# genomicepidemiology/ccphylo

Measured on AMD Instinct MI355X. Metric: taxa-pairs/sec (dist) + NJ iterations/sec at N taxa, 1/2/4/8 MI355X, higher is better.
Workload: dtype u2 packed codes -> MX-fp4 MFMA (exact integer counts), f64 LT and tree

## Files before the change

ccphylo_amd/csrc/ccg_dnj_search.h:

```cpp
#pragma once
#include <stdlib.h>
#include "ccg_tree_common.h"

struct DenseRows {
	__host__ __device__ __forceinline__ bool owns(long long) const { return true; }
	__host__ __device__ __forceinline__ long long row(long long r) const { return tri(r); }
};

#define DNJ_B 128
#define DNJ_BANDS 64
#define DNJ_BANDS_MAX 128
#define SEG 2048
#define SEG_S 1024
#define SEL_RPL 8
#define SEL_STEPS 8
#define TBF 1024
#define FIND_RPT 16
#define FIND_CHUNKS 2048
#define REPLAY_CAP 2048
#define JOIN_UPRE 2048
#define FOLD_BLOCKS 256
#define PLAN_MAXB 256
#define SRDY_REP 64
#define UHIST 64
// ... 116 lines not shown
			const bool take = c < c1 && 0 <= d && qarg_better(x, c, q, idx);
			q = take ? x : q;
			idx = take ? c : idx;
		}
		if(more) {
#pragma unroll
			for(int m = 0; m < UNR; ++m) {
				v[m] = vn[m];
				nk[m] = nkn[m];
				sk[m] = skn[m];
			}
		}
	}
}

__device__ __forceinline__ void fold_units(const double *__restrict__ uq, const int *__restrict__ uj, int ua, int ub,
                                           double &q, int &idx) {
	for(int u = ua; u < ub; u += 4) {
		double oq[4];
		int oi[4];
#pragma unroll
		for(int m = 0; m < 4; ++m) {
			const int v = u + m < ub ? u + m : ub - 1;
			oq[m] = uq[v];
			oi[m] = uj[v];
		}
#pragma unroll
		for(int m = 0; m < 4; ++m) {
			if(u + m < ub && qarg_better(oq[m], oi[m], q, idx)) {
				q = oq[m];
				idx = oi[m];
			}
		}
	}
}

__device__ __forceinline__ void qarg_block_reduce1(double &q, int &idx, double *sq, int *si) {
	qarg_wave_reduce(q, idx);
	const int lane = threadIdx.x & 63, wid = threadIdx.x >> 6, nw = blockDim.x >> 6;
	if(lane == 0) {
		sq[wid] = q;
		si[wid] = idx;
	}
	__syncthreads();
	if(threadIdx.x == 0) {
		for(int w = 1; w < nw; ++w) {
			if(qarg_better(sq[w], si[w], q, idx)) {
				q = sq[w];
				idx = si[w];
			}
		}
	}
}

template <int ET, class Rows>
__global__ void k_init_hnj(Rows rows, const typename Elem<ET>::T *__restrict__ D, int n, double bs,
                           const double *__restrict__ sD, const int *__restrict__ N,
                           double *__restrict__ Q, int *__restrict__ P) {
	int i = blockIdx.x * (blockDim.x >> 6) + (threadIdx.x >> 6);
	int lane = threadIdx.x & 63;
	if(i >= n || !rows.owns(i)) return;
	double bq = DBL_MAX, bd = DBL_MAX;
	int bj = 0;
	const typename Elem<ET>::T *row = D + rows.row(i);
	int Ni = N[i];
	double sDi = sD[i];
	for(int j = lane; j < i; j += 64) {
		double d = Elem<ET>::get(row[j], bs);
		const double q = qcrit(Ni, N[j], d, sDi, sD[j]);
		const bool take = (0 <= d) & ((q < bq) | ((q == bq) & ((d < bd) | ((d == bd) & (j > bj)))));
		bq = take ? q : bq;
		bd = take ? d : bd;
		bj = take ? j : bj;
	}
#pragma unroll
	for(int off = 32; off > 0; off >>= 1) {
		const double oq = __shfl_xor(bq, off, 64), od = __shfl_xor(bd, off, 64);
		const int oj = __shfl_xor(bj, off, 64);
		const bool take = (oq < bq) | ((oq == bq) & ((od < bd) | ((od == bd) & (oj > bj))));
		bq = take ? oq : bq;
		bd = take ? od : bd;
		bj = take ? oj : bj;
	}
	if(lane == 0) {
		Q[i] = bq;
		P[i] = bj;
	}
}

template <int UNUSED = 0>
__global__ __launch_bounds__(TB) void k_dnj_prep(TreeBufs b, int n) {
	__shared__ double sq[TB / 64];
	__shared__ int si[TB / 64];
	double q = DBL_MAX;
	int idx = 0;
	for(int i = 1 + threadIdx.x; i < n; i += blockDim.x) {
		if(qarg_better(b.Q[i], i, q, idx)) {
			q = b.Q[i];
			idx = i;
		}
	}
	qarg_block_reduce(q, idx, sq, si);
	if(threadIdx.x == 0) {
		b.ctl->cand = idx;
		b.ctl->cand_q = b.Q[idx];
		b.ctl->cand_p = b.P[idx];
	}
}

__device__ __forceinline__ void s_table_h(const TreeBufs &b, int n, int nS, double m0) {
	const int lane = threadIdx.x & 63;
	double v[2];
#pragma unroll
	for(int h = 0; h < 2; ++h) {
		const int t = lane + 64 * h;
		v[h] = DBL_MAX;
		if(t < nS) {
			const double f = __hip_atomic_load(b.sfq + t, __ATOMIC_RELAXED, __HIP_MEMORY_SCOPE_AGENT);
			const double qt = __hip_atomic_load(b.pS_q + t, __ATOMIC_RELAXED, __HIP_MEMORY_SCOPE_AGENT);
			v[h] = f > qt ? f : qt;
		}
	}
	double x0 = wave_incl_min(v[0]);
	x0 = x0 < m0 ? x0 : m0;
	const double c = readlane_d(x0, 63);
	double x1 = wave_incl_min(v[1]);
	x1 = x1 < c ? x1 : c;
	if(lane < nS) __hip_atomic_store(b.pS_bnd + lane, x0, __ATOMIC_RELAXED, __HIP_MEMORY_SCOPE_AGENT);
	if(lane + 64 < nS) __hip_atomic_store(b.pS_bnd + lane + 64, x1, __ATOMIC_RELAXED, __HIP_MEMORY_SCOPE_AGENT);
	if(b.ctl->vtag == n) {
		const int G = (int) cdiv(n + 1, TB);
		double carry = DBL_MAX;
		for(int g1 = ((G - 1) / 64) * 64; g1 >= 0; g1 -= 64) {
			const int g = g1 + 63 - lane;
			double x = g < G ? b.bmv[g] : DBL_MAX;
			x = wave_incl_min(x);
			x = x < carry ? x : carry;
			if(g < G) __hip_atomic_store(b.vsuf + g, x, __ATOMIC_RELAXED, __HIP_MEMORY_SCOPE_AGENT);
			carry = readlane_d(x, 63);
		}
		if(lane == 0) __hip_atomic_store(b.vsuf + G, DBL_MAX, __ATOMIC_RELAXED, __HIP_MEMORY_SCOPE_AGENT);
	}
	asm volatile("s_waitcnt vmcnt(0)" ::: "memory");
	if(lane < SRDY_REP)
		__hip_atomic_store(b.srdy + 32 * lane, (unsigned) n, __ATOMIC_RELAXED, __HIP_MEMORY_SCOPE_AGENT);
}

#ifndef LB_BB_D
#define LB_BB_D 8
#endif
#ifndef LB_BB_N
#define LB_BB_N 8
#endif
template <int ET>
__device__ __forceinline__ int lb_unit(const typename Elem<ET>::T *__restrict__ row, double bs, const TreeBufs &b, int n,
                                       int r, int c0, int c1, double sDr, double &q, int &idx, int isub = -1,
                                       double sDm = 0.0, bool ubinf = false);

template <int ET>
__device__ __forceinline__ void plan_s_helper(const typename Elem<ET>::T *__restrict__ D, double bs,
                                                        TreeBufs b, int n, int hb, int nh, bool tshort) {
	typedef typename Elem<ET>::T T;
	constexpr int UC = 8;
	__shared__ int h_ok, h_nS, h_isub, h_jsub;
	__shared__ double h_m0, h_sDm;
	__shared__ int h_uo[DNJ_B + 1], h_row[DNJ_B];
	const int tid = threadIdx.x, lane = tid & 63, wid = tid >> 6;
	if(b.ctl->done) return;
	if(tid == 0) {
		bool ok = false;
		for(int spin = 0; spin < (tshort ? 1 << 10 : 1 << 18); ++spin) {
			if(__hip_atomic_load(b.shdr + 3, __ATOMIC_RELAXED, __HIP_MEMORY_SCOPE_AGENT) == (unsigned long long) n) {
				ok = true;
				break;
			}
			__builtin_amdgcn_s_sleep(4);
		}
		h_ok = ok;
		if(!ok) {
			b.ctl->final_n = -1;
			b.ctl->done = 1;
		}
		if(ok) {
			h_m0 = __longlong_as_double(
			    (long long) __hip_atomic_load(b.shdr + 0, __ATOMIC_RELAXED, __HIP_MEMORY_SCOPE_AGENT));
			h_sDm = __longlong_as_double(
			    (long long) __hip_atomic_load(b.shdr + 1, __ATOMIC_RELAXED, __HIP_MEMORY_SCOPE_AGENT));
			const unsigned long long w = __hip_atomic_load(b.shdr + 2, __ATOMIC_RELAXED, __HIP_MEMORY_SCOPE_AGENT);
			h_nS = (int) (unsigned) (w & 0xffffffffu);
			h_isub = (int) (unsigned) (w >> 32);
			h_jsub = (int) (unsigned) __hip_atomic_load(b.shdr + 4, __ATOMIC_RELAXED, __HIP_MEMORY_SCOPE_AGENT);
		}
	}
	__syncthreads();
	if(!h_ok || h_nS <= 0) return;
	const int nS = h_nS, isub = h_isub, jsub = h_jsub;
	const double sDm = h_sDm;
	for(int t = tid; t <= nS; t += blockDim.x) {
		h_uo[t] = __hip_atomic_load(b.pS_uo + t, __ATOMIC_RELAXED, __HIP_MEMORY_SCOPE_AGENT);
		if(t < nS) h_row[t] = __hip_atomic_load(b.pS_row + t, __ATOMIC_RELAXED, __HIP_MEMORY_SCOPE_AGENT);
	}
	__syncthreads();
	const int su = h_uo[nS];
	const int nwv = blockDim.x >> 6;
	for(int v = hb * nwv + wid; v < su; v += nh * nwv) {
		int lo = 0, hi = nS;
		while(hi - lo > 1) {
			const int mid = (lo + hi) >> 1;
			if(h_uo[mid] <= v) lo = mid; else hi = mid;
		}
		const int r = h_row[lo], c0 = (v - h_uo[lo]) * SEG_S;
		const int c1 = c0 + SEG_S < r ? c0 + SEG_S : r;
		const double sDr = r == isub ? sDm : b.sD[r];
		const T *row = D + tri(r);
		double q = DBL_MAX;
		int idx = 0;
		if(b.lbm) {
			const long long sk = lb_unit<ET>(row, bs, b, n, r, c0, c1, sDr, q, idx, isub, sDm, r == isub || r == jsub);
			if(lane == 0 && sk) {
				long long *slot = b.lbskip + (long long) (LB_SCAN + (hb * nwv + wid) % LB_HELP) * LB_SLOT;
				atomicAdd((unsigned long long *) slot, (unsigned long long) sk);
				atomicAdd((unsigned long long *) (slot + 1), (unsigned long long) sk);
			}
		} else {
			for(int base = c0; base < c1; base += 64 * UC) {
				double sk[UC];
				T vv[UC];
#pragma unroll
				for(int m = 0; m < UC; ++m) {
					const int c = base + 64 * m + lane;
					const int cc = c < c1 ? c : c1 - 1;
					sk[m] = b.sD[cc];
					vv[m] = row[cc];
				}
#pragma unroll
				for(int m = 0; m < UC; ++m) {
					const int c = base + 64 * m + lane;
					const double d = Elem<ET>::get(vv[m], bs);
					const double x = qcrit(n, n, d, sDr, c == isub ? sDm : sk[m]);
					const bool take = c < c1 && 0 <= d && qarg_better(x, c, q, idx);
					q = take ? x : q;
					idx = take ? c : idx;
				}
			}
		}
		qarg_wave_reduce(q, idx);
		int s_done = 0;
		const int ua = h_uo[lo], ub = h_uo[lo + 1];
		int last = 1;
		if(ub - ua > 1) {
			if(lane == 0) {
				__hip_atomic_store(b.uq + v, q, __ATOMIC_RELAXED, __HIP_MEMORY_SCOPE_AGENT);
				__hip_atomic_store(b.uj + v, idx, __ATOMIC_RELAXED, __HIP_MEMORY_SCOPE_AGENT);
				asm volatile("s_waitcnt vmcnt(0)" ::: "memory");
				const unsigned seen = __hip_atomic_fetch_add(b.ecS + lo, 1u, __ATOMIC_RELAXED, __HIP_MEMORY_SCOPE_AGENT);
				last = (int) seen == ub - ua - 1;
				if(last) __hip_atomic_store(b.ecS + lo, 0u, __ATOMIC_RELAXED, __HIP_MEMORY_SCOPE_AGENT);
			}
			last = __shfl(last, 0);
			if(last) {
				for(int x = ua + lane; x < ub; x += 64) {
					const double oq = __hip_atomic_load(b.uq + x, __ATOMIC_RELAXED, __HIP_MEMORY_SCOPE_AGENT);
					const int oi = __hip_atomic_load(b.uj + x, __ATOMIC_RELAXED, __HIP_MEMORY_SCOPE_AGENT);
					if(qarg_better(oq, oi, q, idx)) {
						q = oq;
						idx = oi;
					}
				}
				qarg_wave_reduce(q, idx);
			}
		}
		if(lane == 0) {
			if(last) {
				__hip_atomic_store(b.sfq + lo, q, __ATOMIC_RELAXED, __HIP_MEMORY_SCOPE_AGENT);
				__hip_atomic_store(b.sfj + lo, idx, __ATOMIC_RELAXED, __HIP_MEMORY_SCOPE_AGENT);
				asm volatile("s_waitcnt vmcnt(0)" ::: "memory");
				const unsigned sseen = __hip_atomic_fetch_add(&b.ctl->scnt, 1u, __ATOMIC_RELAXED, __HIP_MEMORY_SCOPE_AGENT);
				s_done = (int) sseen == nS - 1;
				if(s_done) __hip_atomic_store(&b.ctl->scnt, 0u, __ATOMIC_RELAXED, __HIP_MEMORY_SCOPE_AGENT);
			}
		}
		if(__shfl(s_done, 0)) s_table_h(b, n, nS, h_m0);
	}
}

template <int ET, bool GEN, class Rows, bool BANDS>
__global__ __launch_bounds__(TBF) void k_dnj_plan(const typename Elem<ET>::T *__restrict__ D, double bs, TreeBufs b,
                                                  int n, int first, Rows rows, int seg, int ktop, int kbands,
                                                  int qdelay) {
	constexpr int NW = TBF / 64, FR = FIND_RPT, NSP = TBF - 64, LT = TBF - 64, LW = NW - 1;
	__shared__ int sS[DNJ_B];
	__shared__ double sQS[DNJ_B], sQP[DNJ_B];
	__shared__ double spq[NSP];
	__shared__ double spm[DNJ_B + 2];
	__shared__ int s_mw[FR * LW], s_cnt;
	__shared__ double s_sb[LW * FR];
	__shared__ __attribute__((aligned(16))) unsigned char s_sf[LW * FR];
	__shared__ int sch[FIND_CHUNKS];
	__shared__ int s_done, s_isub, s_jsub, s_nS, s_ntop, s_smin, s_Nm;
	__shared__ double s_m0, s_Qj, s_Qi, s_sDm;
	TreeCtl *ctl = b.ctl;
	const int tid = threadIdx.x, lane = tid & 63, wid = tid >> 6;
	const int top = n - 1;
	const int fr = ((qdelay >> 17) & 15) + 1;
	const int nhelp = (qdelay >> 22) & 511;
	if((int) blockIdx.x >= (int) gridDim.x - nhelp) {
// ... 1934 lines not shown
```

ccphylo_amd/csrc/snp.hip:

```cpp
#include <cstring>
#include <vector>
#include <type_traits>
#include "ccg_internal.h"
#include "ccg_shard_layout.h"

#define TILE 128
#define KC 16
#define KCP 8
#define RS 130
#define RSP 130

__device__ __forceinline__ uint32_t xor_or(uint32_t a, uint32_t b, uint32_t c) {
	return __builtin_amdgcn_bitop3_b32(a, b, c, 0xBE);
}

__device__ __forceinline__ uint32_t compress_even(uint64_t x) {
	x &= 0x5555555555555555ull;
	x = (x | (x >> 1)) & 0x3333333333333333ull;
	x = (x | (x >> 2)) & 0x0F0F0F0F0F0F0F0Full;
	x = (x | (x >> 4)) & 0x00FF00FF00FF00FFull;
	x = (x | (x >> 8)) & 0x0000FFFF0000FFFFull;
	x = (x | (x >> 16)) & 0x00000000FFFFFFFFull;
	return (uint32_t) x;
}
// ... 470 lines not shown
				g0[x] = fp4_spread(b[x].x);
			}
#pragma unroll
			for(int ta = 0; ta < 4; ++ta)
#pragma unroll
				for(int tb = 0; tb < 4; ++tb)
					acc[ta][tb] = __builtin_amdgcn_mfma_scale_f32_32x32x64_f8f6f4(
					    f0[ta], g0[tb], acc[ta][tb], MFMA_FP4, MFMA_FP4, 0, MFMA_SCALE1, 0, MFMA_SCALE1);
#pragma unroll
			for(int x = 0; x < 4; ++x) {
				f1[x] = fp4_spread(a[x].y);
				g1[x] = fp4_spread(b[x].y);
			}
#pragma unroll
			for(int ta = 0; ta < 4; ++ta)
#pragma unroll
				for(int tb = 0; tb < 4; ++tb)
					acc[ta][tb] = __builtin_amdgcn_mfma_scale_f32_32x32x64_f8f6f4(
					    f1[ta], g1[tb], acc[ta][tb], MFMA_FP4, MFMA_FP4, 0, MFMA_SCALE1, 0, MFMA_SCALE1);
#pragma unroll
			for(int x = 0; x < 4; ++x) {
				f0[x] = fp4_xor_spread(f0[x], f1[x]);
				g0[x] = fp4_xor_spread(g0[x], g1[x]);
			}
#pragma unroll
			for(int ta = 0; ta < 4; ++ta)
#pragma unroll
				for(int tb = 0; tb < 4; ++tb)
					acc[ta][tb] = __builtin_amdgcn_mfma_scale_f32_32x32x64_f8f6f4(
					    f0[ta], g0[tb], acc[ta][tb], MFMA_FP4, MFMA_FP4, 0, MFMA_SCALE1, 0, MFMA_SCALE1);
		}
		if(more) {
			uint2 *An = As[buf ^ 1], *Bn = Bs[buf ^ 1];
#pragma unroll
			for(int q = 0; q < QS2; ++q) {
				const int e = q * 256 + threadIdx.x, row = e / WPR, wp = e % WPR;
				An[(2 * wp) * RS2 + row] = make_uint2(va[q].x, va[q].y);
				An[(2 * wp + 1) * RS2 + row] = make_uint2(va[q].z, va[q].w);
				Bn[(2 * wp) * RS2 + row] = make_uint2(vb[q].x, vb[q].y);
				Bn[(2 * wp + 1) * RS2 + row] = make_uint2(vb[q].z, vb[q].w);
			}
		}
		__syncthreads();
	}
	const int L3 = 3 * 32 * Wl;
#pragma unroll
	for(int ta = 0; ta < 4; ++ta) {
#pragma unroll
		for(int r = 0; r < 16; ++r) {
			const int l = 128 * wr + 32 * ta + (r & 3) + 8 * (r >> 2) + 4 * h;
			const long long L = (long long) I * TILE2 + l;
			long long i = L;
			if(BAND) {
				const long long lb = L / SB;
				i = (lb * world + rank) * SB + (L - lb * SB);
			}
			if(i >= n || (!BAND && (i < rowBegin || i >= rowEnd))) continue;
			const long long base = BAND ? sh.off(i) : tri(i);
#pragma unroll
			for(int tb = 0; tb < 4; ++tb) {
				const long long j = (long long) J * TILE2 + 128 * wc + 32 * tb + l32;
				if(j < i) {
					const unsigned d = (unsigned) ((L3 - (int) acc[ta][tb][r]) >> 2);
					if(SPLIT) {
						atomicAdd(&cnt[base + j - cbase], d);
					} else {
						const double v = nFactor * (double) d;
						D[base + j] = Elem<ET>::put(v, 0.5, bs);
					}
				}
			}
		}
	}
}

#define NST3 4
#define KC3 8
#ifdef CCG_DIST_STAMPS
#define ST3_SLOTS 8
__device__ unsigned long long *ccg_dist_stamp_buf;
__device__ long long ccg_dist_stamp_item0;
#define ST3(K)                                                                              \
	do {                                                                                    \
		unsigned long long tn_;                                                             \
		__builtin_amdgcn_sched_barrier(0);                                                  \
		asm volatile("s_memtime %0\n\ts_waitcnt lgkmcnt(0)" : "=s"(tn_)::"memory");         \
		__builtin_amdgcn_sched_barrier(0);                                                  \
		if((K) >= 0) stamp_sum[(K) < 0 ? 0 : (K)] += tn_ - stamp_prev;                      \
		stamp_prev = tn_;                                                                   \
	} while(0)
#else
#define ST3(K)
#endif
template <int ET, bool SPLIT, bool BAND>
__global__ __launch_bounds__(256, 1) void k_snp_mfma3(const uint2 *__restrict__ P, int Wp, int n, long long t0,
                                                      long long items, int S, int Wk, double nFactor, double bs,
                                                      typename Elem<ET>::T *__restrict__ D, long long rowBegin,
                                                      long long rowEnd, unsigned *__restrict__ cnt, long long cbase,
                                                      const long long *__restrict__ pfx, int npanels, int rank,
                                                      int world, int sorder) {
	constexpr int NSL = KC3 / 2;
	static_assert(NSL == 4, "one slice per wave");
	__shared__ __attribute__((aligned(16))) uint4 L[NST3 * 2 * NSL * TILE2];
	const long long item = t0 + xcd_tile(blockIdx.x, items), t = SPLIT ? item / S : item;
	int I, J;
	if(BAND) {
		int lo = 0, hi = npanels - 1;
		while(lo < hi) {
			const int mid = (lo + hi + 1) >> 1;
			if(pfx[mid] <= t) lo = mid; else hi = mid - 1;
		}
		I = lo;
		J = (int) (t - pfx[lo]);
	} else if(sorder) {
		tile_ij_super(t, (rowEnd - 1) / TILE2, I, J);
	} else {
		tile_ij(t, I, J);
	}
	const int wb = SPLIT ? (int) (item % S) * Wk : 0;
	const int Wl = SPLIT ? (wb + Wk < Wp ? Wk : Wp - wb) : Wp;
	const Shard sh{rank, world};
	const int lane = threadIdx.x & 63, wid = threadIdx.x >> 6;
	const uint2 *srcA[4], *srcB[4];
#pragma unroll
	for(int q = 0; q < 4; ++q) {
		const long long Lr = (long long) I * TILE2 + q * 64 + lane;
		long long r = Lr;
		if(BAND) {
			const long long lb = Lr / SB;
			r = (lb * world + rank) * SB + (Lr - lb * SB);
			r = r < n ? r : 0;
		}
		srcA[q] = P + (size_t) r * Wp + wb + 2 * wid;
		srcB[q] = P + ((size_t) J * TILE2 + q * 64 + lane) * Wp + wb + 2 * wid;
	}
	const int nch = Wl / KC3;
	const unsigned lbase = (unsigned) (uintptr_t) (__attribute__((address_space(3))) uint4 *) L;
	auto glds = [&](const uint2 *src, unsigned lds) {
		unsigned keep;
		asm volatile("s_mov_b32 %0, m0\n\ts_mov_b32 m0, %2\n\ts_nop 0\n\tglobal_load_lds_dwordx4 %1, off\n\ts_mov_b32 m0, %0"
		             : "=&s"(keep)
		             : "v"(src), "s"(lds)
		             : "memory");
	};
	const unsigned lwave = (unsigned) __builtin_amdgcn_readfirstlane((int) (lbase + (unsigned) (wid * TILE2 * 16)));
	auto issue1 = [&](int c, int i) {
		const int st = c % NST3, w0 = c * KC3, q = i >> 1, p = i & 1;
		glds((p ? srcB[q] : srcA[q]) + w0, lwave + (unsigned) ((((st * 2 + p) * NSL) * TILE2 + q * 64) * 16));
	};
	auto issue = [&](int c) {
#pragma unroll
		for(int i = 0; i < 8; ++i) issue1(c, i);
	};
	const int wr = wid >> 1, wc = wid & 1;
	const int h = lane >> 5, l32 = lane & 31;
	const int ra0 = 128 * wr + l32, rb0 = 128 * wc + l32;
	v16f_t acc[4][4];
#pragma unroll
	for(int ta = 0; ta < 4; ++ta)
#pragma unroll
		for(int tb = 0; tb < 4; ++tb)
#pragma unroll
			for(int r = 0; r < 16; ++r) acc[ta][tb][r] = 0.0f;
	auto land = [&](int c) {
		const int ahead = nch - 1 - c < NST3 - 2 ? nch - 1 - c : NST3 - 2;
		if(ahead >= 2) asm volatile("s_waitcnt vmcnt(16)" ::: "memory");
		else if(ahead == 1) asm volatile("s_waitcnt vmcnt(8)" ::: "memory");
		else asm volatile("s_waitcnt vmcnt(0)" ::: "memory");
		asm volatile("" ::: "memory");
		__builtin_amdgcn_s_barrier();
		asm volatile("" ::: "memory");
	};
	auto rd1 = [&](int gs, int p, uint2 (&v)[4]) {
		const int st = (gs >> 2) % NST3, sl = gs & 3;
		const uint2 *Pc = (const uint2 *) &L[((st * 2 + p) * NSL + sl) * TILE2];
#pragma unroll
		for(int x = 0; x < 4; ++x) v[x] = Pc[((p ? rb0 : ra0) + 32 * x) * 2 + h];
	};
	auto rd = [&](int gs, uint2 (&a)[4], uint2 (&b)[4]) {
		rd1(gs, 0, a);
		rd1(gs, 1, b);
	};
#define MF3(TA, TB, F, G)                                                                                         \
	acc[TA][TB] = __builtin_amdgcn_mfma_scale_f32_32x32x64_f8f6f4(F, G, acc[TA][TB], MFMA_FP4, MFMA_FP4, 0, MFMA_SCALE1, \
	                                                              0, MFMA_SCALE1)
	for(int c = 0; c < NST3 - 1 && c < nch; ++c) issue(c);
	land(0);
	if(NST3 - 1 < nch) issue(NST3 - 1);
	uint2 a[4], b[4];
	v8i_t f0[4], g0[4];
	rd(0, a, b);
#pragma unroll
	for(int x = 0; x < 4; ++x) {
		f0[x] = fp4_spread(a[x].x);
		g0[x] = fp4_spread(b[x].x);
	}
#ifdef CCG_DIST_STAMPS
	unsigned long long stamp_sum[ST3_SLOTS] = {0, 0, 0, 0, 0, 0, 0, 0}, stamp_prev = 0;
#endif
#define GAP3() __builtin_amdgcn_sched_barrier(0)
	auto step = [&](auto OPEN, auto MORE, int gs) {
		constexpr int open = decltype(OPEN)::value;
		constexpr bool more = decltype(MORE)::value;
		v8i_t f1[4], g1[4], x0[4], y0[4];
#pragma unroll
		for(int k = 0; k < 16; ++k) {
			MF3(k >> 2, k & 3, f0[k >> 2], g0[k & 3]);
			const int j = k >> 1;
			if(j == 0 || j > 4) fp4_spread_half(f1[j ? j - 4 : 0], a[j ? j - 4 : 0].y, k & 1);
			else fp4_spread_half(g1[j - 1], b[j - 1].y, k & 1);
			GAP3();
		}
		const int cn = (gs + 1) >> 2;
		if(open) {
			ST3(3);
			GAP3();
			if(open == 2) {
				asm volatile("s_waitcnt vmcnt(16)" ::: "memory");
				asm volatile("" ::: "memory");
				__builtin_amdgcn_s_barrier();
				asm volatile("" ::: "memory");
			} else {
				land(cn);
			}
			GAP3();
			ST3(4);
		}
		uint2 an[4], bn[4];
#pragma unroll
		for(int k = 0; k < 16; ++k) {
			MF3(k >> 2, k & 3, f1[k >> 2], g1[k & 3]);
			const int j = k >> 1;
			if(j == 0 || j > 4) fp4_xor_spread_half(x0[j ? j - 4 : 0], f0[j ? j - 4 : 0], f1[j ? j - 4 : 0], k & 1);
			else fp4_xor_spread_half(y0[j - 1], g0[j - 1], g1[j - 1], k & 1);
			if(more && k == 0) rd1(gs + 1, 0, an);
			if(more && k == 1) rd1(gs + 1, 1, bn);
			if(open == 2 && (k & 1)) issue1(cn + NST3 - 1, k >> 1);
			GAP3();
		}
		if(open == 2) ST3(5);
#pragma unroll
		for(int k = 0; k < 16; ++k) {
			MF3(k >> 2, k & 3, x0[k >> 2], y0[k & 3]);
			if(more) {
				const int j = k >> 1;
				if(j == 0 || j > 4) fp4_spread_half(f0[j ? j - 4 : 0], an[j ? j - 4 : 0].x, k & 1);
				else fp4_spread_half(g0[j - 1], bn[j - 1].x, k & 1);
			}
			GAP3();
		}
		if(more) {
#pragma unroll
			for(int x = 0; x < 4; ++x) {
				a[x] = an[x];
				b[x] = bn[x];
			}
		}
	};
	typedef std::integral_constant<int, 0> O0;
	typedef std::integral_constant<int, 1> O1;
	typedef std::integral_constant<int, 2> O2;
	typedef std::true_type MT;
	ST3(-1);
	int c = 0;
	for(; c + NST3 < nch; ++c) {
		step(O0(), MT(), 4 * c + 0);
		ST3(0);
		step(O0(), MT(), 4 * c + 1);
		ST3(1);
		step(O0(), MT(), 4 * c + 2);
		ST3(2);
		step(O2(), MT(), 4 * c + 3);
		ST3(6);
	}
	for(; c + 1 < nch; ++c) {
		step(O0(), MT(), 4 * c + 0);
		step(O0(), MT(), 4 * c + 1);
		step(O0(), MT(), 4 * c + 2);
		step(O1(), MT(), 4 * c + 3);
	}
#ifdef CCG_DIST_STAMPS
	if(ccg_dist_stamp_buf && lane == 0 && (wid == 0 || wid == 3)) {
		stamp_sum[7] = nch > NST3 ? nch - NST3 : 0;
		unsigned long long *sb =
		    ccg_dist_stamp_buf + ((t0 - ccg_dist_stamp_item0 + blockIdx.x) * 2 + (wid ? 1 : 0)) * ST3_SLOTS;
		for(int k = 0; k < ST3_SLOTS; ++k) sb[k] = stamp_sum[k];
	}
#endif
	{
		const int g = 4 * (nch - 1);
		step(O0(), MT(), g + 0);
		step(O0(), MT(), g + 1);
		step(O0(), MT(), g + 2);
		step(O0(), std::false_type(), g + 3);
	}
#undef MF3
#undef GAP3
	const int L3 = 3 * 32 * Wl;
#pragma unroll
	for(int ta = 0; ta < 4; ++ta) {
#pragma unroll
		for(int r = 0; r < 16; ++r) {
			const int l = 128 * wr + 32 * ta + (r & 3) + 8 * (r >> 2) + 4 * h;
			const long long Lr = (long long) I * TILE2 + l;
			long long i = Lr;
			if(BAND) {
				const long long lb = Lr / SB;
				i = (lb * world + rank) * SB + (Lr - lb * SB);
			}
			if(i >= n || (!BAND && (i < rowBegin || i >= rowEnd))) continue;
			const long long base = BAND ? sh.off(i) : tri(i);
#pragma unroll
			for(int tb = 0; tb < 4; ++tb) {
				const long long j = (long long) J * TILE2 + 128 * wc + 32 * tb + l32;
				if(j < i) {
					const unsigned d = (unsigned) ((L3 - (int) acc[ta][tb][r]) >> 2);
					if(SPLIT) {
						atomicAdd(&cnt[base + j - cbase], d);
					} else {
						const double v = nFactor * (double) d;
						D[base + j] = Elem<ET>::put(v, 0.5, bs);
					}
				}
			}
		}
	}
}

template <int ET>
__global__ void k_snp_finish(const unsigned *__restrict__ cnt, long long cbase, long long f0, long long f1,
                             double nFactor, double bs, typename Elem<ET>::T *__restrict__ D) {
	for(long long f = f0 + (long long) blockIdx.x * blockDim.x + threadIdx.x; f < f1;
	    f += (long long) gridDim.x * blockDim.x) {
		D[f] = Elem<ET>::put(nFactor * (double) cnt[f - cbase], 0.5, bs);
	}
}

template <int ET>
__device__ __forceinline__ void pair_store(typename Elem<ET>::T *D, typename Elem<ET>::T *N, long long f, uint32_t dist,
                                           uint32_t inc, unsigned norm, unsigned minLength, double bs) {
	typedef typename Elem<ET>::T T;
	if(ET == 8) {
		double v;
		if(minLength <= inc) {
			v = norm ? (double) ((unsigned long long) dist * norm) / inc : (double) dist;
		} else {
			v = -1.0;
		}
		D[f] = (T) v;
		if(N) N[f] = (T) (double) inc;
	} else if(ET == 4) {
		float v;
		if(minLength <= inc) {
			if(norm) {
				v = (float) ((unsigned long long) dist * norm);
				v = v / (float) inc;
			} else {
				v = (float) dist;
			}
		} else {
			v = -1.0f;
		}
		D[f] = (T) v;
		if(N) N[f] = (T) (float) inc;
	} else {
		double v;
		if(minLength <= inc) {
			v = norm ? ((double) ((unsigned long long) dist * norm) * bs + 0.5) / inc : (double) dist * bs + 0.5;
		} else {
			v = -1.0 * bs + 0;
		}
		D[f] = (T) cvt_i32_x86(v);
		if(N) N[f] = (T) cvt_i32_x86(inc * bs + 0.5);
	}
}

template <int ET, bool SPLIT, bool BAND>
__global__ __launch_bounds__(256, 2) void k_snp_tile_pair(const uint4 *__restrict__ P, int Wp, int n, long long t0,
                                                          long long items, int S, int Wk, unsigned norm,
                                                          unsigned minLength, double bs,
                                                          typename Elem<ET>::T *__restrict__ D,
                                                          typename Elem<ET>::T *__restrict__ Nm, long long rowBegin,
                                                          long long rowEnd, unsigned *__restrict__ cd,
                                                          unsigned *__restrict__ cn, long long cbase,
                                                          const long long *__restrict__ pfx, int npanels, int rank,
                                                          int world) {
	__shared__ __attribute__((aligned(16))) uint4 As[2][KCP * RSP];
	__shared__ __attribute__((aligned(16))) uint4 Bs[2][KCP * RSP];
	int I, J;
	const long long item = t0 + xcd_tile(blockIdx.x, items);
	if(BAND) band_ij(pfx, npanels, item / S, I, J);
	else tile_ij(item / S, I, J);
	const Shard sh{rank, world};
	const int wb = (int) (item % S) * Wk, we = wb + Wk < Wp ? wb + Wk : Wp;
	const int Wl = we - wb;
	const int tx = threadIdx.x & 15, ty = threadIdx.x >> 4;
	const uint4 *Aq[4];
#pragma unroll
	for(int q = 0; q < 4; ++q) {
		const long long L = (long long) I * TILE + ((q * 256 + threadIdx.x) >> 3);
		Aq[q] = P + (size_t) (BAND ? band_row(sh, L, n) : L) * Wp + wb;
	}
	const uint4 *Bp = P + (size_t) J * TILE * Wp + wb;
	uint32_t ad[8][8], an[8][8];
#pragma unroll
	for(int a = 0; a < 8; ++a)
#pragma unroll
		for(int c = 0; c < 8; ++c) {
			ad[a][c] = 0;
			an[a][c] = 0;
		}
	uint4 va[4], vb[4];
#pragma unroll
	for(int q = 0; q < 4; ++q) {
		const int e = q * 256 + threadIdx.x, row = e >> 3, wp = e & 7;
		va[q] = Aq[q][wp];
		vb[q] = Bp[(size_t) row * Wp + wp];
	}
#pragma unroll
	for(int q = 0; q < 4; ++q) {
		const int e = q * 256 + threadIdx.x, row = e >> 3, wp = e & 7;
		As[0][wp * RSP + row] = va[q];
		Bs[0][wp * RSP + row] = vb[q];
	}
	__syncthreads();
	int buf = 0;
	for(int w0 = 0; w0 < Wl; w0 += KCP, buf ^= 1) {
		const bool more = w0 + KCP < Wl;
		if(more) {
#pragma unroll
			for(int q = 0; q < 4; ++q) {
				const int e = q * 256 + threadIdx.x, row = e >> 3, wp = e & 7;
				va[q] = Aq[q][w0 + KCP + wp];
				vb[q] = Bp[(size_t) row * Wp + w0 + KCP + wp];
			}
		}
		const uint4 *Ac = As[buf], *Bc = Bs[buf];
#pragma unroll 1
		for(int w = 0; w < KCP; ++w) {
			uint4 a[8], b[8];
#pragma unroll
			for(int q = 0; q < 4; ++q) {
				a[2 * q] = Ac[w * RSP + 2 * ty + 32 * q];
				a[2 * q + 1] = Ac[w * RSP + 2 * ty + 32 * q + 1];
				b[2 * q] = Bc[w * RSP + 2 * tx + 32 * q];
				b[2 * q + 1] = Bc[w * RSP + 2 * tx + 32 * q + 1];
			}
// ... 1069 lines not shown
```

ccphylo_amd/csrc/tree.hip:

```cpp
#include <string.h>
#include <stdio.h>
#include <vector>
#include <stdlib.h>
#include "ccg_tree_common.h"

#include "ccg_dnj_search.h"

static thread_local DnjGrid g_grid;

template <int ET>
__global__ __launch_bounds__(TB) void k_init_rows(const typename Elem<ET>::T *__restrict__ D, int n, double bs,
                                                  double *__restrict__ sD, int *__restrict__ N, TreeCtl *ctl) {
	__shared__ double buf[TB / 64][64];
	const int lane = threadIdx.x & 63, wid = threadIdx.x >> 6;
	const int k = blockIdx.x * (TB / 64) + wid;
	if(k >= n) return;
	double s = 0;
	int c = 1, miss = 0;
	const typename Elem<ET>::T *row = D + tri(k);
	for(int m0 = 0; m0 < k; m0 += 64) {
		int m = m0 + lane;
		double d = m < k ? Elem<ET>::get(row[m], bs) : 0.0;
		bool ok = m < k && 0 <= d;
		miss |= m < k && !ok;
// ... 1674 lines not shown
				switch(sm) {
#define SV_(M) case 4 + M: k_dnj_scan_v<ET, DenseRows, FoldTail, M, true><<<gc, TB, 0, st>>>(D, bs, b, n, DenseRows(), seg); break;
					SV_(1) SV_(5)
#undef SV_
					default: k_dnj_scan_v<ET, DenseRows, FoldTail, 0, true><<<gc, TB, 0, st>>>(D, bs, b, n, DenseRows(), seg);
				}
			} else if(tfold) {
				switch(sm) {
#define SV_(M) case 4 + M: k_dnj_scan_v<ET, DenseRows, FoldTail, M><<<gc, TB, 0, st>>>(D, bs, b, n, DenseRows(), seg); break;
					SV_(1) SV_(5)
#undef SV_
					default: k_dnj_scan_v<ET, DenseRows, FoldTail><<<gc, TB, 0, st>>>(D, bs, b, n, DenseRows(), seg);
				}
			} else {
				switch(sm) {
#define SV_(M) case 4 + M: k_dnj_scan_v<ET, DenseRows, NoTail, M><<<gc, TB, 0, st>>>(D, bs, b, n, DenseRows(), seg); break;
					SV_(1) SV_(2) SV_(3) SV_(4) SV_(5) SV_(6) SV_(7) SV_(13) SV_(15)
#undef SV_
					default: k_dnj_scan_v<ET, DenseRows><<<gc, TB, 0, st>>>(D, bs, b, n, DenseRows(), seg);
				}
			}
		} else if(sm >= 1) {
			if(tfold) k_dnj_scan_w<ET, GEN, DenseRows, FoldTail><<<gc, TB, 0, st>>>(D, bs, b, n, DenseRows(), seg);
			else k_dnj_scan_w<ET, GEN><<<gc, TB, 0, st>>>(D, bs, b, n, DenseRows(), seg);
		} else k_dnj_scan<ET, GEN><<<gc, TB, 0, st>>>(D, bs, b, n, DenseRows(), seg);
		if(prefold && !tfold) k_dnj_fold<><<<FOLD_BLOCKS, TB, 0, st>>>(b, n, seg, prune == 2);
		kt.mark(CCG_K_REST);
		if(prefold && g_grid.join_pf) k_dnj_join_pf<ET, GEN><<<gn, TB, 0, st>>>(D, bs, b, n, general, g_grid.join_pf == 2);
		else k_dnj_join<ET, GEN><<<gn, TB, 0, st>>>(D, bs, b, n, general, prefold, seg);
		if(GEN) k_update_general<ET><<<1, 1024, 0, st>>>(D, bs, b, n);
		kt.mark(CCG_K_UPDATE);
		if(xs) {
			k_exact_sum<><<<1, XS_NT, 0, st>>>(b, n, (int) gn);
			kt.mark(CCG_K_XSUM);
		}
		if(g_grid.bands(n - 1) && g_grid.scan_vblk && dnj_prune(n - 1, ET, GEN))
			k_dnj_requeue<ET, true, true><<<gn, TB, 0, st>>>(D, bs, b, n, general, exact);
		else if(g_grid.bands(n - 1)) k_dnj_requeue<ET, true><<<gn, TB, 0, st>>>(D, bs, b, n, general, exact);
		else k_dnj_requeue<ET, false><<<gn, TB, 0, st>>>(D, bs, b, n, general, exact);
		kt.mark(CCG_K_REQUEUE);
		return (GEN ? 5 : 4) + (prefold && !tfold) + (prune == 2) + xs;
	}
	if(method == CCG_TREE_HNJ) {
		k_hnj_argmin<><<<gn, TB, 0, st>>>(b, n);
		kt.mark(CCG_K_ARGMIN);
		k_nj_join<ET><<<gn, TB, 0, st>>>(D, bs, b, n, (int) gn, general, DBL_MAX);
		if(GEN) k_update_general<ET><<<1, 1024, 0, st>>>(D, bs, b, n);
		kt.mark(CCG_K_UPDATE);
		if(xs) {
			k_exact_sum<><<<1, XS_NT, 0, st>>>(b, n, (int) gn);
			kt.mark(CCG_K_XSUM);
		}
		k_hnj_update<ET><<<gn, TB, 0, st>>>(D, bs, b, n, general, exact);
		kt.mark(CCG_K_POP);
		return (GEN ? 4 : 3) + xs;
	}
	const unsigned g = (unsigned) nj_blocks(n);
	if(method == CCG_TREE_MN) k_nj_argmin<ET, GEN, true><<<g, TB, 0, st>>>(D, bs, b, n);
	else k_nj_argmin<ET, GEN><<<g, TB, 0, st>>>(D, bs, b, n);
	kt.mark(CCG_K_ARGMIN);
	k_nj_join<ET><<<gn, TB, 0, st>>>(D, bs, b, n, (int) g, general, method == CCG_TREE_MN ? DBL_MAX : 1.0);
	if(GEN) k_update_general<ET><<<1, 1024, 0, st>>>(D, bs, b, n);
	kt.mark(CCG_K_UPDATE);
	if(xs) {
		k_exact_sum<><<<1, XS_NT, 0, st>>>(b, n, (int) gn);
		kt.mark(CCG_K_XSUM);
	}
	k_nj_pop<ET><<<gn, TB, 0, st>>>(D, b, n, general, exact);
	kt.mark(CCG_K_POP);
	return (GEN ? 4 : 3) + xs;
}

static bool g_progress = false;

template <int ET>
static int tree_run_t(ccg_ctx *ctx, const ccg_tree_args *a, void *Dd, ccg_join *joins, int *njoins,
                      int *final_n, double *final_d, int64_t *stats, const ccg_dnj_state *sin,
                      ccg_dnj_state *sout) {
	typedef typename Elem<ET>::T T;
	T *D = (T *) Dd;
	const int n0 = a->n;
	const double bs = a->byteScale;
	hipStream_t st = ctx->stream;
	TreeWork w;
	g_grid = DnjGrid();
	g_grid.load();
	g_progress = getenv("CCG_PROGRESS") != nullptr;
	const bool cmp_env = getenv("CCG_SCAN_CMPB") != nullptr;
	auto cmp_share = [&](int blocks) {
		return ctx->cus > 0 && ctx->cus < ctx->ncu ? (blocks * ctx->cus / ctx->ncu > 64 ? blocks * ctx->cus / ctx->ncu : 64)
		                                           : blocks;
	};
	if(!cmp_env) g_grid.cmp_blocks = cmp_share(g_grid.cmp_blocks);
	int rc = tree_alloc_ctx(ctx, &w, n0);
	if(rc) return rc;
	TreeBufs b = w.b;
	TreeCtl init;
	memset(&init, 0, sizeof(init));
	init.neg = (a->flags & 2) != 0;
	init.exact = a->exact != 0;
	init.method = a->method;
	init.hj = init.hi = -1;
	if(sin) {
		init.cand = sin->cand;
		init.cand_q = sin->Q[sin->cand];
		init.cand_p = sin->P[sin->cand];
	}
	CCG_CHECK(hipMemcpyAsync(b.ctl, &init, sizeof(init), hipMemcpyHostToDevice, st));
	long long launches = 0;
	static thread_local KTimer kt;
	CCG_CHECK(hipEventRecord(ctx->ev0, st));
	kt.init(st, a->profile != 0);
	k_init_rows<ET><<<cdiv(n0, TB / 64), TB, 0, st>>>(D, n0, bs, b.sD, b.N, b.ctl);
	k_init_cols<ET><<<cdiv(n0, TB), TB, 0, st>>>(D, n0, bs, b.sD, b.N, b.ctl);
	launches += 2;
	bool resumed_counts = false;
	if(sin) {
		CCG_CHECK(hipMemcpyAsync(b.sD, sin->sD, (size_t) n0 * 8, hipMemcpyHostToDevice, st));
		CCG_CHECK(hipMemcpyAsync(b.Q, sin->Q, (size_t) n0 * 8, hipMemcpyHostToDevice, st));
		CCG_CHECK(hipMemcpyAsync(b.N, sin->N, (size_t) n0 * 4, hipMemcpyHostToDevice, st));
		CCG_CHECK(hipMemcpyAsync(b.P, sin->P, (size_t) n0 * 4, hipMemcpyHostToDevice, st));
		for(int k = 0; k < n0 && !resumed_counts; ++k) resumed_counts = sin->N[k] != n0;
	} else if(a->method == CCG_TREE_DNJ) {
		k_init_hnj<ET><<<cdiv(n0, TB / 64), TB, 0, st>>>(DenseRows(), D, n0, bs, b.sD, b.N, b.Q, b.P);
		k_dnj_prep<><<<1, TB, 0, st>>>(b, n0);
		launches += 2;
	} else if(a->method == CCG_TREE_HNJ) {
		k_init_hnj<ET><<<cdiv(n0, TB / 64), TB, 0, st>>>(DenseRows(), D, n0, bs, b.sD, b.N, b.Q, b.P);
		launches += 1;
	}
	kt.mark(CCG_K_INIT);
	CCG_CHECK(hipGetLastError());
	TreeCtl h;
	CCG_CHECK(hipMemcpyAsync(&h, b.ctl, sizeof(h), hipMemcpyDeviceToHost, st));
	CCG_CHECK(hipStreamSynchronize(st));
	const bool general = h.has_missing != 0 || resumed_counts;
	void *lbmem = NULL;
	if(a->method == CCG_TREE_DNJ && !general && g_grid.lb && n0 > g_grid.lb_min_n) {
		const long long LS = (n0 + LBW - 1) / LBW;
		const size_t lbb = ((size_t) n0 * LS * 4 + 255) & ~(size_t) 255;
		const size_t msb = ((size_t) (LS + 1) * 8 + 255) & ~(size_t) 255;
		const size_t ubb = ((size_t) n0 * 8 + 255) & ~(size_t) 255, skb = (size_t) (LB_SCAN + LB_HELP) * LB_SLOT * 8;
		if(ccg_ctx_workspace(ctx, 1, lbb + msb + ubb + skb, &lbmem) == CCG_OK) {
			b.lbm = (unsigned *) lbmem;
			b.msd = (double *) ((char *) lbmem + lbb);
			b.ubq = (double *) ((char *) lbmem + lbb + msb);
			b.lbs = LS;
			b.lbskip = (long long *) ((char *) lbmem + lbb + msb + ubb);
			CCG_CHECK(hipMemsetAsync(b.lbskip, 0, skb, st));
			k_lb_init<ET><<<cdiv(n0, TB / 64), TB, 0, st>>>(D, n0, bs, b);
			launches += 1;
			CCG_CHECK(hipGetLastError());
			if(!getenv("CCG_SCAN_PRUNE")) g_grid.scan_prune = 0;
			if(!cmp_env) g_grid.cmp_blocks = cmp_share(2048);
		} else {
			(void) hipGetLastError();
			lbmem = NULL;
		}
	}
#ifdef CCG_TRACE
	const char *tn = getenv("CCG_TRACE_N");
	int trace_hi = tn ? atoi(tn) : n0 / 2;
	CCG_CHECK(hipMemcpyToSymbolAsync(HIP_SYMBOL(g_trace_hi), &trace_hi, sizeof(int), 0, hipMemcpyHostToDevice, st));
	static unsigned long long zero_tr[256 * 4 * 16];
	CCG_CHECK(hipMemcpyToSymbolAsync(HIP_SYMBOL(g_trace), zero_tr, sizeof(zero_tr), 0, hipMemcpyHostToDevice, st));
#endif
	int n = n0;
	int since_check = 0;
	long long win_rows = h.rows, win_cells = h.cells;
	bool stopped = false;
	const int stop_n = a->max_joins > 0 && a->max_joins < n0 - 2 ? n0 - a->max_joins : 2;
	while(n > stop_n) {
		launches += general ? enqueue_iteration<ET, true>(st, D, bs, b, n, n == n0, a->method, a->exact, kt)
		                    : enqueue_iteration<ET, false>(st, D, bs, b, n, n == n0, a->method, a->exact, kt);
		CCG_CHECK(hipGetLastError());
		--n;
		if(++since_check == 1024) {
			since_check = 0;
			CCG_CHECK(hipMemcpyAsync(&h, b.ctl, sizeof(h), hipMemcpyDeviceToHost, st));
			CCG_CHECK(hipStreamSynchronize(st));
			g_grid.small_wave = g_grid.adapt_rows && h.rows - win_rows > 1024LL * g_grid.adapt_rows;
			g_grid.prune_on = !g_grid.prune_cells || h.cells - win_cells > 1024LL * g_grid.prune_cells;
			win_rows = h.rows;
			win_cells = h.cells;
			if(g_progress && (n0 - n) % (16 * 1024) == 0)
				fprintf(stderr, "ccg_tree: %d joins, n = %d, rows %lld cells %lld (reference rule %lld / %lld)\n", n0 - n,
				        n, h.rows, h.cells, h.ref_rows, h.ref_cells);
			if(h.done) {
				stopped = true;
				break;
			}
		}
	}
	(void) stopped;
	CCG_CHECK(hipEventRecord(ctx->ev1, st));
	kt.finish();
	CCG_CHECK(hipMemcpyAsync(&h, b.ctl, sizeof(h), hipMemcpyDeviceToHost, st));
	CCG_CHECK(hipStreamSynchronize(st));
	if(b.lbskip) {
		std::vector<long long> sl((size_t) (LB_SCAN + LB_HELP) * LB_SLOT);
		CCG_CHECK(hipMemcpyAsync(sl.data(), b.lbskip, sl.size() * 8, hipMemcpyDeviceToHost, st));
		CCG_CHECK(hipStreamSynchronize(st));
		for(size_t x = 0; x < (size_t) LB_SCAN + LB_HELP; ++x) {
			h.cells_lbskip += sl[x * LB_SLOT];
			h.cells_help -= sl[x * LB_SLOT + 1];
		}
	}
	float ms = 0;
	CCG_CHECK(hipEventElapsedTime(&ms, ctx->ev0, ctx->ev1));
	if(getenv("CCG_XS_WHY"))
		fprintf(stderr, "xs_why: value %d nc %d nt %d stuck %d ex0 %d cap %d walk %d (chain sums %d of %d)\n",
		        h.xs_why[0], h.xs_why[1], h.xs_why[2], h.xs_why[3], h.xs_why[4], h.xs_why[5], h.xs_why[6],
		        h.chain_sums, h.serial_sums);
#ifdef CCG_TRACE
	{
		static unsigned long long tr[256 * NKT * 16];
		CCG_CHECK(hipMemcpyFromSymbol(tr, HIP_SYMBOL(g_trace), sizeof(tr), 0, hipMemcpyDeviceToHost));
		const int nk = a->method == CCG_TREE_DNJ ? NKT : 0;
		double acc[NKT][16] = {{0}}, gap[NKT] = {0}, itv = 0;
		int cnt = 0;
		bool present[NKT] = {false};
		for(int s = 0; s < 256; ++s)
			for(int k = 0; k < nk; ++k) present[k] = present[k] || tr[(s * NKT + k) * 16 + 15];
		for(int s = 0; s < 256; ++s) {
			const unsigned long long *e = tr + s * NKT * 16;
			bool ok = true;
			for(int k = 0; k < nk; ++k) ok = ok && (!present[k] || (e[k * 16 + 15] && e[k * 16 + 14]));
			if(!ok) continue;
			++cnt;
			int k0 = 0, prev = -1;
			while(k0 < nk && !present[k0]) ++k0;
			for(int k = k0; k < nk; ++k) {
				if(!present[k]) continue;
				unsigned long long t0 = ~e[k * 16 + 15];
				for(int p = 0; p < 15; ++p)
					if(e[k * 16 + p]) acc[k][p] += ((double) e[k * 16 + p] - (double) t0) / 100.0;
				if(prev >= 0) gap[k] += ((double) t0 - (double) e[prev * 16 + 14]) / 100.0;
				prev = k;
			}
			if(s + 1 < 256 && tr[((s + 1) * NKT + k0) * 16 + 15]) {
				gap[k0] += ((double) ~tr[((s + 1) * NKT + k0) * 16 + 15] - (double) e[(nk - 1) * 16 + 14]) / 100.0;
				itv += ((double) ~tr[((s + 1) * NKT + k0) * 16 + 15] - (double) ~e[k0 * 16 + 15]) / 100.0;
			}
		}
		const char *kn[NKT] = {"select", "plan/find", "scan", "join", "requeue"};
		fprintf(stderr, "trace: %d joins at n <= %d; iteration %.2f us; serial replays %d, serial sums %d\n", cnt,
		        trace_hi, cnt ? itv / (cnt - 1) : 0, h.serial_replays, h.serial_sums);
		{
			static unsigned long long sp[256 * 64 * 3];
			CCG_CHECK(hipMemcpyFromSymbol(sp, HIP_SYMBOL(g_samp), sizeof(sp), 0, hipMemcpyDeviceToHost));
			double st_max = 0, en_max = 0, dur = 0, st_med = 0, stg = 0;
			int sc = 0, jc = 0;
			for(int s = 0; s < 256; ++s) {
				const unsigned long long t0 = ~tr[(s * NKT + 2) * 16 + 15];
				if(!tr[(s * NKT + 2) * 16 + 15]) continue;
				double smax = 0, emax = 0;
				int any = 0;
				for(int q = 0; q < 64; ++q) {
					const unsigned long long *e = sp + (s * 64 + q) * 3;
					if(!e[0] || !e[2] || e[0] < t0) continue;
					const double a = (e[0] - t0) / 100.0, z = (e[2] - t0) / 100.0;
					smax = a > smax ? a : smax;
					emax = z > emax ? z : emax;
					dur += z - a;
					if(e[1] >= e[0]) stg += (e[1] - e[0]) / 100.0;
					st_med += a;
					++sc;
					any = 1;
				}
				if(any) {
					st_max += smax;
					en_max += emax;
					++jc;
				}
			}
			{
				static unsigned long long ua[256 * 64 * 8];
				CCG_CHECK(hipMemcpyFromSymbol(ua, HIP_SYMBOL(g_uamp), sizeof(ua), 0, hipMemcpyDeviceToHost));
				double ud[4] = {0}, ug[4] = {0}, us0 = 0;
				int uc[4] = {0}, gc[4] = {0}, s0c = 0;
				for(int s = 0; s < 256; ++s) {
					const unsigned long long t0 = ~tr[(s * NKT + 2) * 16 + 15];
					if(!tr[(s * NKT + 2) * 16 + 15]) continue;
					for(int q = 0; q < 64; ++q) {
						const unsigned long long *e = ua + (s * 64 + q) * 8;
						const unsigned long long *sp0 = sp + (s * 64 + q) * 3;
						if(e[0] && e[0] >= t0 && sp0[0] && e[0] >= sp0[0]) {
							us0 += (e[0] - sp0[0]) / 100.0;
							++s0c;
						}
						for(int k = 0; k < 4; ++k) {
							if(e[2 * k] && e[2 * k + 1] >= e[2 * k] && e[2 * k] >= t0) {
								ud[k] += (e[2 * k + 1] - e[2 * k]) / 100.0;
								++uc[k];
							}
							if(k && e[2 * k] && e[2 * k - 1] && e[2 * k] >= e[2 * k - 1] && e[2 * k] >= t0) {
								ug[k] += (e[2 * k] - e[2 * k - 1]) / 100.0;
								++gc[k];
							}
						}
					}
				}
				fprintf(stderr, "  scan units (wave 0 of sampled blocks): entry->first unit %.2f us;", s0c ? us0 / s0c : 0.0);
				for(int k = 0; k < 4; ++k)
					fprintf(stderr, " unit%d n=%d dur %.2f gap %.2f;", k, uc[k], uc[k] ? ud[k] / uc[k] : 0.0, gc[k] ? ug[k] / gc[k] : 0.0);
				fprintf(stderr, "\n");
				memset(ua, 0, sizeof(ua));
// ... 149 lines not shown
```

Baseline: 200.2 million.

## Spread next-chunk LDS loads across steps and size LB scan grid by occupancy

The FP4 MFMA distance kernel used to issue all eight global_load_lds pieces of the next pipeline chunk inside a single step. It now spreads them across several steps through a carry state: two pieces go out in the opening step and the rest are carried into the following chunk's first steps, with pointer advances done incrementally. This is meant to even out VMEM issue pressure among the MFMA work and avoid bursts that stall the matrix pipe, at the cost of extra template variants and more complex vmcnt accounting. Separately, the DNJ lower-bound scan grid size now comes from the HIP occupancy query times the CU count times two rounds, replacing a fixed share of 2048.

```diff
diff --git a/ccphylo_amd/csrc/ccg_dnj_search.h b/ccphylo_amd/csrc/ccg_dnj_search.h
--- a/ccphylo_amd/csrc/ccg_dnj_search.h
+++ b/ccphylo_amd/csrc/ccg_dnj_search.h
@@ -292,6 +292,7 @@
 #ifndef LB_BB_N
 #define LB_BB_N 8
 #endif
+#define LB_GRID_ROUNDS 2
 template <int ET>
 __device__ __forceinline__ int lb_unit(const typename Elem<ET>::T *__restrict__ row, double bs, const TreeBufs &b, int n,
                                        int r, int c0, int c1, double sDr, double &q, int &idx, int isub = -1,
diff --git a/ccphylo_amd/csrc/snp.hip b/ccphylo_amd/csrc/snp.hip
--- a/ccphylo_amd/csrc/snp.hip
+++ b/ccphylo_amd/csrc/snp.hip
@@ -646,6 +646,14 @@
 #pragma unroll
 		for(int i = 0; i < 8; ++i) issue1(c, i);
 	};
+	auto piece = [&](int c, int i) {
+		const int st = c % NST3, q = i >> 1, p = i & 1;
+		glds(p ? srcB[q] : srcA[q], lwave + (unsigned) ((((st * 2 + p) * NSL) * TILE2 + q * 64) * 16));
+	};
+	auto advance = [&](int i) {
+		if(i & 1) srcB[i >> 1] += KC3;
+		else srcA[i >> 1] += KC3;
+	};
 	const int wr = wid >> 1, wc = wid & 1;
 	const int h = lane >> 5, l32 = lane & 31;
 	const int ra0 = 128 * wr + l32, rb0 = 128 * wc + l32;
@@ -681,6 +689,13 @@
 	for(int c = 0; c < NST3 - 1 && c < nch; ++c) issue(c);
 	land(0);
 	if(NST3 - 1 < nch) issue(NST3 - 1);
+	if(NST3 < nch) {
+#pragma unroll
+		for(int q = 0; q < 4; ++q) {
+			srcA[q] += NST3 * KC3;
+			srcB[q] += NST3 * KC3;
+		}
+	}
 	uint2 a[4], b[4];
 	v8i_t f0[4], g0[4];
 	rd(0, a, b);
@@ -693,9 +708,12 @@
 	unsigned long long stamp_sum[ST3_SLOTS] = {0, 0, 0, 0, 0, 0, 0, 0}, stamp_prev = 0;
 #endif
 #define GAP3() __builtin_amdgcn_sched_barrier(0)
-	auto step = [&](auto OPEN, auto MORE, int gs) {
-		constexpr int open = decltype(OPEN)::value;
+#define PGAP3 7
+	auto step = [&](auto OPEN, auto MORE, auto CARRY, int gs) {
+		constexpr int open = decltype(OPEN)::value, carry = decltype(CARRY)::value;
 		constexpr bool more = decltype(MORE)::value;
+		static_assert(!(open == 2 && carry), "a step opens the next chunk's pieces or carries the last one's");
+		const int cp = (gs >> 2) + NST3 - 1;
 		v8i_t f1[4], g1[4], x0[4], y0[4];
 #pragma unroll
 		for(int k = 0; k < 16; ++k) {
@@ -703,6 +721,7 @@
 			const int j = k >> 1;
 			if(j == 0 || j > 4) fp4_spread_half(f1[j ? j - 4 : 0], a[j ? j - 4 : 0].y, k & 1);
 			else fp4_spread_half(g1[j - 1], b[j - 1].y, k & 1);
+			if((carry == 1 || carry == 2) && k == PGAP3) piece(cp, 3 * carry - 1);
 			GAP3();
 		}
 		const int cn = (gs + 1) >> 2;
@@ -729,7 +748,9 @@
 			else fp4_xor_spread_half(y0[j - 1], g0[j - 1], g1[j - 1], k & 1);
 			if(more && k == 0) rd1(gs + 1, 0, an);
 			if(more && k == 1) rd1(gs + 1, 1, bn);
-			if(open == 2 && (k & 1)) issue1(cn + NST3 - 1, k >> 1);
+			if(open == 2 && k == PGAP3) piece(cn + NST3 - 1, 0);
+			if((carry == 1 || carry == 2) && k == PGAP3) piece(cp, 3 * carry);
+			if(carry == 3 && k >= 2 && k < 10) advance(k - 2);
 			GAP3();
 		}
 		if(open == 2) ST3(5);
@@ -741,6 +762,8 @@
 				if(j == 0 || j > 4) fp4_spread_half(f0[j ? j - 4 : 0], an[j ? j - 4 : 0].x, k & 1);
 				else fp4_spread_half(g0[j - 1], bn[j - 1].x, k & 1);
 			}
+			if(open == 2 && k == PGAP3) piece(cn + NST3 - 1, 1);
+			if((carry == 1 || carry == 2) && k == PGAP3) piece(cp, 3 * carry + 1);
 			GAP3();
 		}
 		if(more) {
@@ -755,23 +778,41 @@
 	typedef std::integral_constant<int, 1> O1;
 	typedef std::integral_constant<int, 2> O2;
 	typedef std::true_type MT;
+	typedef std::integral_constant<int, 1> C1;
+	typedef std::integral_constant<int, 2> C2;
+	typedef std::integral_constant<int, 3> C3;
 	ST3(-1);
 	int c = 0;
-	for(; c + NST3 < nch; ++c) {
-		step(O0(), MT(), 4 * c + 0);
+	if(NST3 < nch) {
+		step(O0(), MT(), O0(), 0);
 		ST3(0);
-		step(O0(), MT(), 4 * c + 1);
+		step(O0(), MT(), O0(), 1);
 		ST3(1);
-		step(O0(), MT(), 4 * c + 2);
+		step(O0(), MT(), O0(), 2);
 		ST3(2);
-		step(O2(), MT(), 4 * c + 3);
+		step(O2(), MT(), O0(), 3);
 		ST3(6);
+		for(c = 1; c + NST3 < nch; ++c) {
+			step(O0(), MT(), C1(), 4 * c + 0);
+			ST3(0);
+			step(O0(), MT(), C2(), 4 * c + 1);
+			ST3(1);
+			step(O0(), MT(), C3(), 4 * c + 2);
+			ST3(2);
+			step(O2(), MT(), O0(), 4 * c + 3);
+			ST3(6);
+		}
+		step(O0(), MT(), C1(), 4 * c + 0);
+		step(O0(), MT(), C2(), 4 * c + 1);
+		step(O0(), MT(), O0(), 4 * c + 2);
+		step(O1(), MT(), O0(), 4 * c + 3);
+		++c;
 	}
 	for(; c + 1 < nch; ++c) {
-		step(O0(), MT(), 4 * c + 0);
-		step(O0(), MT(), 4 * c + 1);
-		step(O0(), MT(), 4 * c + 2);
-		step(O1(), MT(), 4 * c + 3);
+		step(O0(), MT(), O0(), 4 * c + 0);
+		step(O0(), MT(), O0(), 4 * c + 1);
+		step(O0(), MT(), O0(), 4 * c + 2);
+		step(O1(), MT(), O0(), 4 * c + 3);
 	}
 #ifdef CCG_DIST_STAMPS
 	if(ccg_dist_stamp_buf && lane == 0 && (wid == 0 || wid == 3)) {
@@ -783,10 +824,10 @@
 #endif
 	{
 		const int g = 4 * (nch - 1);
-		step(O0(), MT(), g + 0);
-		step(O0(), MT(), g + 1);
-		step(O0(), MT(), g + 2);
-		step(O0(), std::false_type(), g + 3);
+		step(O0(), MT(), O0(), g + 0);
+		step(O0(), MT(), O0(), g + 1);
+		step(O0(), MT(), O0(), g + 2);
+		step(O0(), std::false_type(), O0(), g + 3);
 	}
 #undef MF3
 #undef GAP3
diff --git a/ccphylo_amd/csrc/tree.hip b/ccphylo_amd/csrc/tree.hip
--- a/ccphylo_amd/csrc/tree.hip
+++ b/ccphylo_amd/csrc/tree.hip
@@ -1850,7 +1850,14 @@
 			launches += 1;
 			CCG_CHECK(hipGetLastError());
 			if(!getenv("CCG_SCAN_PRUNE")) g_grid.scan_prune = 0;
-			if(!cmp_env) g_grid.cmp_blocks = cmp_share(2048);
+			if(!cmp_env) {
+				int res = 0;
+				CCG_CHECK(hipOccupancyMaxActiveBlocksPerMultiprocessor(
+				    &res, k_dnj_scan_v<ET, DenseRows, NoTail, 0, 0, true, true>, TB, 0));
+				const int cus = ctx->cus > 0 && ctx->cus < ctx->ncu ? ctx->cus : ctx->ncu;
+				const long long g = (long long) res * cus * LB_GRID_ROUNDS;
+				g_grid.cmp_blocks = (int) (g < 64 ? 64 : g);
+			}
 		} else {
 			(void) hipGetLastError();
 			lbmem = NULL;
```

Measured after the change: 200.4 million (median of 5 runs). About the same (+0.1%).
